# zhaoruiyang98/eftpipe

Hardware: AMD Instinct MI355X
Metric: theory P_l(k) evaluations/sec (single tracer, Nk=512, l=0,2,4) (higher is better)
Workload: dtype f64

## Files before the change

### eftpipe_amd/csrc/eftb_kernels.hpp

```cpp
#pragma once
#include <hip/hip_runtime.h>
#include <stdint.h>
#include <stdlib.h>

namespace eftb {

constexpr int NS = 80;
constexpr int NPOW = 257;
constexpr int NHALF = 128;
constexpr int NCH = 129;

constexpr int NROW = 24;

typedef double v4d __attribute__((ext_vector_type(4)));
typedef double v2d __attribute__((ext_vector_type(2)));

__device__ __forceinline__ void xcd_decode(int ntile, int& tile, int& group) {
    const int flat = blockIdx.x, ng = gridDim.x / ntile;
    if ((ng & 7) == 0) {
        const int slot = flat >> 3;
        tile = slot % ntile;
        group = (flat & 7) + 8 * (slot / ntile);
    } else {
        tile = flat % ntile;
// ... 74 lines not shown
__device__ __forceinline__ void qf_body(int w, int nq, const double* __restrict__ fgrow, const double* __restrict__ Qpoly, double* __restrict__ Q) {
    const int tid = threadIdx.x;
    const double f = fgrow[w];
    for (int idx = tid; idx < 2 * nq; idx += blockDim.x) {
        const int a = idx / nq, rest = idx % nq;
        const double* c = Qpoly + ((size_t)(1 - a) * nq + rest) * 15;
        double cv[15];
#pragma unroll
        for (int p = 0; p < 15; ++p) cv[p] = c[p];
        const double f2 = f * f;
        double ev = cv[14], od = cv[13];
#pragma unroll
        for (int p = 12; p >= 0; p -= 2) {
            ev = fma(ev, f2, cv[p]);
            if (p >= 1) od = fma(od, f2, cv[p - 1]);
        }
        Q[(size_t)w * 2 * nq + idx] = fma(od, f, ev);
    }
}

__global__ __launch_bounds__(256) void prep_rows_qf_kernel(int B, PREP_ROWS_PARAMS, int nq, const double* __restrict__ fgrow,
                                                           const double* __restrict__ Qpoly, double* __restrict__ Q) {
    if ((int)blockIdx.x >= B) {
        qf_body(blockIdx.x - B, nq, fgrow, Qpoly, Q);
        return;
    }
    prep_rows_body<false>(PREP_ROWS_ARGS, 0, 0);
}

__global__ __launch_bounds__(256) void prep_rows_qf_lo_kernel(int B, PREP_ROWS_PARAMS, int nq, const double* __restrict__ fgrow,
                                                              const double* __restrict__ Qpoly, double* __restrict__ Q, int ntail_lo, int nxtail_lo) {
    if ((int)blockIdx.x >= B) {
        qf_body(blockIdx.x - B, nq, fgrow, Qpoly, Q);
        return;
    }
    prep_rows_body<true>(PREP_ROWS_ARGS, ntail_lo, nxtail_lo);
}
#undef PREP_ROWS_PARAMS
#undef PREP_ROWS_ARGS

constexpr int AD_T = NHALF + 2;
constexpr int AD_CH = 1;
constexpr int KSYN = 528;
constexpr int KLIN = 288;
constexpr int SYN_KPAD = 48;
constexpr int SYN_KC = 24;
static_assert(SYN_KPAD % SYN_KC == 0 && (32 * SYN_KC) % 256 == 0, "chunk must divide the padding and fill the staging threads");
constexpr int BAS22 = 8, BASC = 32;

__device__ __forceinline__ double readlane_f64(double v, int lane) {
    return __hiloint2double(__builtin_amdgcn_readlane(__double2hiint(v), lane), __builtin_amdgcn_readlane(__double2loint(v), lane));
}

template <int NC, int NW>
__global__ __launch_bounds__(64 * NW) void antidiag_kernel(int B, int Bmax, const double* __restrict__ coefT,
                                                           const double2* __restrict__ AD, double2* __restrict__ S) {
    constexpr int PB = 3, WPP = 2 * NC;
    static_assert(PB * WPP <= 64, "one wave-load must hold a block's weights");
    __shared__ double red[NW - 1][2 * NC][64];
    const int grp = blockIdx.y, jp = (grp & 1) ? NPOW - 1 - (int)blockIdx.x : (int)blockIdx.x;
    const int lane = threadIdx.x & 63, wave = threadIdx.x >> 6, w = grp * 64 + lane;
    const int wl = w < B ? w : B - 1;
    const int cnt = ((2 * NHALF + jp) >> 1) - jp + 1;
    const int per = (cnt + NW - 1) / NW, t0 = wave * per, t1 = min(cnt, t0 + per);
    const double* cr = coefT + wl;
    const double* ci = coefT + (size_t)NCH * Bmax + wl;
    double ar[NC], ai[NC];
#pragma unroll
    for (int q = 0; q < NC; ++q) ar[q] = ai[q] = 0.0;
    if (t0 < t1) {
        const double* adw = reinterpret_cast<const double*>(AD + ((size_t)jp * AD_T + t0) * NC);
        const int nw = (t1 - t0) * WPP;
        auto wload = [&](int blk) { return adw[min(blk * PB * WPP + lane, nw - 1)]; };
        double xr[PB], xi[PB], yr[PB], yi[PB];
        auto coef = [&](int t, int p) {
            const int n = jp + t, qn = n <= NHALF ? n : 2 * NHALF - n;
            xr[p] = cr[(size_t)qn * Bmax];
            xi[p] = ci[(size_t)qn * Bmax];
            yr[p] = cr[(size_t)t * Bmax];
            yi[p] = ci[(size_t)t * Bmax];
        };
        double wc = wload(0);
#pragma unroll
        for (int p = 0; p < PB; ++p) coef(min(t0 + p, t1 - 1), p);
        const int nblk = (t1 - t0 + PB - 1) / PB;
        for (int blk = 0; blk < nblk; ++blk) {
            const double wn = wload(blk + 1);
#pragma unroll
            for (int p = 0; p < PB; ++p) {
                const int t = t0 + blk * PB + p;
                const double on = t < t1 ? 1.0 : 0.0;
                const double xim = jp + t <= NHALF ? xi[p] : -xi[p], yim = -yi[p];
                const double pr = (xr[p] * yr[p] - xim * yim) * on, pi = (xr[p] * yim + xim * yr[p]) * on;
                __builtin_amdgcn_sched_barrier(0);
                coef(min(t + PB, t1 - 1), p);
                __builtin_amdgcn_sched_barrier(0);
#pragma unroll
                for (int q = 0; q < NC; ++q) {
                    const double mx = readlane_f64(wc, p * WPP + 2 * q), my = readlane_f64(wc, p * WPP + 2 * q + 1);
                    ar[q] = fma(mx, pr, fma(-my, pi, ar[q]));
                    ai[q] = fma(mx, pi, fma(my, pr, ai[q]));
                }
                __builtin_amdgcn_sched_barrier(0);
            }
            wc = wn;
        }
    }
    if (wave > 0) {
#pragma unroll
        for (int q = 0; q < NC; ++q) {
            red[wave - 1][2 * q][lane] = ar[q];
            red[wave - 1][2 * q + 1][lane] = ai[q];
        }
    }
    __syncthreads();
    if (wave == 0 && w < B) {
#pragma unroll
        for (int q = 0; q < NC; ++q) {
#pragma unroll
            for (int v = 0; v < NW - 1; ++v) {
                ar[q] += red[v][2 * q][lane];
                ai[q] += red[v][2 * q + 1][lane];
            }
            S[((size_t)w * NC + q) * NPOW + jp] = make_double2(ar[q], ai[q]);
        }
    }
}

template <int NC, int NW>
__global__ __launch_bounds__(64 * NW) void antidiag_nh_kernel(int B, int Bmax, const double* __restrict__ coefT,
                                                              const double2* __restrict__ AD, double2* __restrict__ S, int nh) {
    constexpr int PB = 3, WPP = 2 * NC;
    static_assert(PB * WPP <= 64, "one wave-load must hold a block's weights");
    __shared__ double red[NW - 1][2 * NC][64];
    const int npow = 2 * nh + 1, nch = nh + 1, adt = nh + 2;
    const int grp = blockIdx.y, jp = (grp & 1) ? npow - 1 - (int)blockIdx.x : (int)blockIdx.x;
    const int lane = threadIdx.x & 63, wave = threadIdx.x >> 6, w = grp * 64 + lane;
    const int wl = w < B ? w : B - 1;
    const int cnt = ((2 * nh + jp) >> 1) - jp + 1;
    const int per = (cnt + NW - 1) / NW, t0 = wave * per, t1 = min(cnt, t0 + per);
    const double* cr = coefT + wl;
    const double* ci = coefT + (size_t)nch * Bmax + wl;
    double ar[NC], ai[NC];
#pragma unroll
    for (int q = 0; q < NC; ++q) ar[q] = ai[q] = 0.0;
    if (t0 < t1) {
        const double* adw = reinterpret_cast<const double*>(AD + ((size_t)jp * adt + t0) * NC);
        const int nw = (t1 - t0) * WPP;
        auto wload = [&](int blk) { return adw[min(blk * PB * WPP + lane, nw - 1)]; };
        double xr[PB], xi[PB], yr[PB], yi[PB];
        auto coef = [&](int t, int p) {
            const int n = jp + t, qn = n <= nh ? n : 2 * nh - n;
            xr[p] = cr[(size_t)qn * Bmax];
            xi[p] = ci[(size_t)qn * Bmax];
            yr[p] = cr[(size_t)t * Bmax];
            yi[p] = ci[(size_t)t * Bmax];
        };
        double wc = wload(0);
#pragma unroll
        for (int p = 0; p < PB; ++p) coef(min(t0 + p, t1 - 1), p);
        const int nblk = (t1 - t0 + PB - 1) / PB;
        for (int blk = 0; blk < nblk; ++blk) {
            const double wn = wload(blk + 1);
#pragma unroll
            for (int p = 0; p < PB; ++p) {
                const int t = t0 + blk * PB + p;
                const double on = t < t1 ? 1.0 : 0.0;
                const double xim = jp + t <= nh ? xi[p] : -xi[p], yim = -yi[p];
                const double pr = (xr[p] * yr[p] - xim * yim) * on, pi = (xr[p] * yim + xim * yr[p]) * on;
                __builtin_amdgcn_sched_barrier(0);
                coef(min(t + PB, t1 - 1), p);
                __builtin_amdgcn_sched_barrier(0);
#pragma unroll
                for (int q = 0; q < NC; ++q) {
                    const double mx = readlane_f64(wc, p * WPP + 2 * q), my = readlane_f64(wc, p * WPP + 2 * q + 1);
                    ar[q] = fma(mx, pr, fma(-my, pi, ar[q]));
                    ai[q] = fma(mx, pi, fma(my, pr, ai[q]));
                }
                __builtin_amdgcn_sched_barrier(0);
            }
            wc = wn;
        }
    }
    if (wave > 0) {
#pragma unroll
        for (int q = 0; q < NC; ++q) {
            red[wave - 1][2 * q][lane] = ar[q];
            red[wave - 1][2 * q + 1][lane] = ai[q];
        }
    }
    __syncthreads();
    if (wave == 0 && w < B) {
#pragma unroll
        for (int q = 0; q < NC; ++q) {
#pragma unroll
            for (int v = 0; v < NW - 1; ++v) {
                ar[q] += red[v][2 * q][lane];
                ai[q] += red[v][2 * q + 1][lane];
            }
            S[((size_t)w * NC + q) * npow + jp] = make_double2(ar[q], ai[q]);
        }
    }
}

template <int NC>
__global__ __launch_bounds__(64) void build_rows_kernel(int sets, int Bmax, int Nl, int nlc, int nb, const double* __restrict__ coef,
                                                         const double2* __restrict__ S, const double2* __restrict__ mlj,
                                                         const double2* __restrict__ linvec, double* __restrict__ A22,
                                                         double* __restrict__ A13, double* __restrict__ ACF, double* __restrict__ ALC) {
    const int w = blockIdx.x, cf = blockIdx.y, jp = blockIdx.z * 64 + threadIdx.x;
    if (((sets >> cf) & 1) && jp < NPOW) {
        double zr[NC], zi[NC];
#pragma unroll
        for (int q = 0; q < NC; ++q) {
            zr[q] = zi[q] = 0.0;
#pragma unroll
            for (int ch = 0; ch < AD_CH; ++ch) {
                const double2 v = S[(((size_t)ch * Bmax + w) * NC + q) * NPOW + jp];
                zr[q] += v.x;
                zi[q] += v.y;
            }
        }
        const int o0 = jp == 0 ? 0 : 2 * jp - 1;
        if (cf == 0) {
#pragma unroll
            for (int q = 0; q < NC; ++q)
                if (q < nb) {
                    double* o = A22 + ((size_t)w * BAS22 + q) * KSYN;
                    o[o0] = zr[q];
                    if (jp) o[o0 + 1] = zi[q];
                }
        } else {
            for (int l = 0; l < Nl; ++l) {
                const double2 m = mlj[l * NPOW + jp];
#pragma unroll
                for (int q = 0; q < NC; ++q) {
                    double* o = ACF + ((size_t)w * BASC + l * NC + q) * KSYN;
                    o[o0] = m.x * zr[q] - m.y * zi[q];
                    if (jp) o[o0 + 1] = m.x * zi[q] + m.y * zr[q];
                }
            }
        }
    }
    if ((sets >> (2 + cf)) & 1) {
        const int nrows = cf == 0 ? 10 : nlc * Nl, v0 = cf == 0 ? 0 : 10;
        double* out = cf == 0 ? A13 + (size_t)w * 10 * KLIN : ALC + (size_t)w * nlc * Nl * KLIN;
        const double* c = coef + (size_t)w * 2 * NCH;
        for (int e = jp; e < nrows * NCH; e += 320) {
            const int row = e / NCH, mp = e % NCH, n = NHALF - mp;
            const double2 v = linvec[(size_t)(v0 + row) * NCH + n];
            const double cr = c[n], ci = n == NHALF ? 0.0 : c[NCH + n];
            double* o = out + (size_t)row * KLIN;
            if (mp == 0) o[0] = cr * v.x - ci * v.y;
            else {
                o[2 * mp - 1] = cr * v.x - ci * v.y;
// ... 4175 lines not shown
```

### eftpipe_amd/csrc/eftbird.hip

```cpp
#include "../../include/eftbird.h"

#include <hip/hip_runtime.h>
#include <dlfcn.h>
#include <rccl/rccl.h>

#include <algorithm>
#include <array>
#include <atomic>
#include <chrono>
#include <cmath>
#include <condition_variable>
#include <mutex>
#include <thread>
#include <cstdarg>
#include <cstdint>
#include <cstdio>
#include <cstdlib>
#include <cstring>
#include <functional>
#include <memory>
#include <string>
#include <tuple>
#include <algorithm>
#include <vector>
// ... 333 lines not shown
    ncclResult_t (*Send)(const void*, size_t, ncclDataType_t, int, ncclComm_t, hipStream_t) = nullptr;
    ncclResult_t (*Recv)(void*, size_t, ncclDataType_t, int, ncclComm_t, hipStream_t) = nullptr;
    const char* (*GetErrorString)(ncclResult_t) = nullptr;
};
static RcclApi g_rccl;

static int rccl_load() {
    if (g_rccl.handle) return 0;
    void* h = dlopen("librccl.so.1", RTLD_NOW | RTLD_GLOBAL);
    if (!h) h = dlopen("librccl.so", RTLD_NOW | RTLD_GLOBAL);
    if (!h) return fail("cannot load librccl.so: %s", dlerror());
#define RSYM(field, name)                                                 \
    g_rccl.field = reinterpret_cast<decltype(g_rccl.field)>(dlsym(h, name)); \
    if (!g_rccl.field) return fail("librccl.so lacks %s", name);
    RSYM(GetUniqueId, "ncclGetUniqueId")
    RSYM(CommInitRank, "ncclCommInitRank")
    RSYM(CommDestroy, "ncclCommDestroy")
    RSYM(GroupStart, "ncclGroupStart")
    RSYM(GroupEnd, "ncclGroupEnd")
    RSYM(Send, "ncclSend")
    RSYM(Recv, "ncclRecv")
    RSYM(GetErrorString, "ncclGetErrorString")
#undef RSYM
    g_rccl.handle = h;
    return 0;
}

#define NCCLCHK(expr)                                                                            \
    do {                                                                                         \
        ncclResult_t _r = (expr);                                                                \
        if (_r != ncclSuccess) return fail("%s failed: %s", #expr, g_rccl.GetErrorString(_r));   \
    } while (0)

static inline void trace_point(eftb_engine* e, int p, hipStream_t st) {
    if (e->trace_slot >= 0) (void)hipEventRecord(e->evTrace[e->trace_slot][p], st);
}

static inline size_t kpad(int n) { return (size_t)(n + SYN_KPAD - 1) / SYN_KPAD * SYN_KPAD; }

static inline int cfg_nh(const eftb_config& c) { return c.nfft ? c.nfft / 2 : NHALF; }
static inline int cfg_npow(const eftb_config& c) { return 2 * cfg_nh(c) + 1; }
static inline int cfg_nch(const eftb_config& c) { return cfg_nh(c) + 1; }

static size_t need_table_bytes(const eftb_config& c, int id) {
    const size_t D = sizeof(double);
    const int Nn = 2 * c.NIR * c.Na;
    switch (id) {
        case EFTB_T_K: return D * c.Nk;
        case EFTB_T_S: return D * NS;
        case EFTB_T_LNKIN: return D * c.Nkin;
        case EFTB_T_SKT: return D * kpad(c.Nkin) * c.Nk;
        case EFTB_T_GCT: case EFTB_T_ECT: return D * kpad(c.Nkin + c.ntail) * 2 * cfg_nch(c);
        case EFTB_T_LNXTAIL: return D * c.ntail;
        case EFTB_T_AD: return 2 * D * (size_t)(c.nbasis + (c.with_resum ? c.nbasis13 : 0)) * cfg_npow(c) * (cfg_nh(c) + 2);
        case EFTB_T_EXP22: return D * 28 * BAS22;
        case EFTB_T_EXPC: return c.with_resum ? D * (size_t)c.Nl * 38 * BASC : 0;
        case EFTB_T_MLJ: return c.with_resum ? 2 * D * c.Nl * cfg_npow(c) : 0;
        case EFTB_T_LINVEC: return 2 * D * (size_t)(10 + (c.with_resum ? (c.with_nnlo ? 3 : 2) * c.Nl : 0)) * cfg_nch(c);
        case EFTB_T_SYNK: return D * (size_t)ksyn_of(cfg_nh(c)) * c.Nk;
        case EFTB_T_LINK: return D * (size_t)klin_of(cfg_nh(c)) * c.Nk;
        case EFTB_T_SYNS: return c.with_resum ? D * (size_t)ksyn_of(cfg_nh(c)) * NS : 0;
        case EFTB_T_LINS: return c.with_resum ? D * (size_t)klin_of(cfg_nh(c)) * NS : 0;
        case EFTB_T_L11: return D * c.Nl * 3;
        case EFTB_T_LCT: return D * c.Nl * 6;
        case EFTB_T_L22: return D * c.Nl * 28;
        case EFTB_T_L13: return D * c.Nl * 10;
        case EFTB_T_GRP: return sizeof(int32_t) * 38 * 2;
        case EFTB_T_BXT: return c.with_resum ? D * kpad(c.Nkin + c.nxtail) * 2 * NS : 0;
        case EFTB_T_TYT: return 0;
        case EFTB_T_LNXXTAIL: return c.with_resum ? D * c.nxtail : 0;
        case EFTB_T_WQLAST2: return c.with_resum ? D * (c.nxtail_lo ? 4 : 2) : 0;
        case EFTB_T_QPOLY: return c.with_resum ? D * 2 * c.Nl * c.Nl * Nn * 15 : 0;
        case EFTB_T_H: return c.with_resum ? D * c.Na * NS * c.Nk : 0;
        case EFTB_T_RSBASIS: case EFTB_T_RSBASISS: return c.with_resum ? D * RS_NB * 16 : 0;
        case EFTB_T_RSROWS: return c.with_resum ? sizeof(int32_t) * 2 * RS3_ROWS : 0;
        case EFTB_T_MU: case EFTB_T_WMU: return c.with_ap ? D * c.nmu : 0;
        case EFTB_T_LEGMU: return c.with_ap ? D * c.Nl * c.nmu : 0;
        case EFTB_T_SPBAND: return c.with_ap ? D * (size_t)(2 * SPL_HB + 1) * c.Nk : 0;
        case EFTB_T_SPCBAND: return c.with_ap ? D * (size_t)(2 * SPL_HB + 1) * c.Nk : 0;
        case EFTB_T_SPLOCAL: return c.with_ap ? D * (size_t)16 * c.Nk : 0;
        case EFTB_T_APFID: return c.with_ap ? D * 2 : 0;
        case EFTB_T_LCTN: return c.with_nnlo ? D * c.Nl * 6 : 0;
        case EFTB_T_BAO: return c.optiresum && c.with_resum ? D * (2 * NS + 4) : 0;
        case EFTB_T_GCT2: case EFTB_T_GCT2T: return c.dual_coef ? D * kpad(c.Nkin + c.ntail) * 2 * cfg_nch(c) : 0;
        case EFTB_T_QEPOLY: return c.with_resum && c.Nl == 3 ? D * 2 * c.Nl * c.Nl * RSD_NN * 15 : 0;
    }
    return 0;
}

static size_t need_buffer_elems(const eftb_config& c, int id) {
    const size_t B = c.max_batch;
    const int Nn = 2 * c.NIR * c.Na;
    switch (id) {
        case EFTB_B_PIN: return B * c.Nkin;
        case EFTB_B_F: case EFTB_B_DA: case EFTB_B_H: return B;
        case EFTB_B_P11: return B * c.Nk;
        case EFTB_B_P22: return B * 28 * c.Nk;
        case EFTB_B_P13: return B * 10 * c.Nk;
        case EFTB_B_C11: case EFTB_B_CCT: return c.with_resum ? B * c.Nl * NS : 0;
        case EFTB_B_CC: return c.with_resum ? B * c.Nl * 38 * NS : 0;
        case EFTB_B_CLOOPL: return c.with_resum ? B * c.Nl * 12 * NS : 0;
        case EFTB_B_TEMPL: return B * c.Nl * NROW * c.Nk;
        case EFTB_B_XY: return c.with_resum ? B * 2 * NS : 0;
        case EFTB_B_Q: return c.with_resum ? B * 2 * c.Nl * c.Nl * Nn : 0;
        case EFTB_B_BIAS: return B * NROW;
        case EFTB_B_PLK: return B * c.Nl * c.Nk;
        case EFTB_B_COEF: return B * 2 * cfg_nch(c);
// ... 2 lines not shown
        case EFTB_B_CCTN: return c.with_nnlo && c.with_resum ? B * c.Nl * NS : 0;
        case EFTB_B_TEMPLN: return c.with_nnlo ? B * c.Nl * NROW * c.Nk : 0;
        case EFTB_B_BIASN: return c.with_nnlo ? B * 3 : 0;
        case EFTB_B_GROWSN: return c.with_nnlo ? B * MARG_NG1 * 3 : 0;
    }
    return 0;
}

template <typename T>
static inline const T* tb(const eftb_engine* e, int id) { return static_cast<const T*>(e->tab[id]); }

static void queue_synth(SynthBatch& sb, const double* A, long long a_group, int groups, int rpg, int K, const double* Tab, int X, double* out,
                        long long o_group, const double* gscale, const double* xscale) {
    SynthDesc& d = sb.p[sb.n];
    d.A = A; d.Tab = Tab; d.out = out; d.gscale = gscale; d.xscale = xscale;
    d.a_group = a_group; d.o_group = o_group; d.M = groups * rpg; d.rpg = rpg; d.K = K; d.X = X;
    d.wgx = (X + 63) / 64;
    d.wg_end = (sb.n ? sb.p[sb.n - 1].wg_end : 0) + d.wgx * ((d.M + 31) / 32);
    ++sb.n;
}

static void launch_synth(hipStream_t st, const SynthBatch& sb) {
    if (sb.n) hipLaunchKernelGGL(synth_kernel, dim3(sb.p[sb.n - 1].wg_end), dim3(256), 0, st, sb);
}

static void launch_gemm_direct(hipStream_t st, SynthBatch sb) {
    int end = 0;
    for (int i = 0; i < sb.n; ++i) {
        SynthDesc& d = sb.p[i];
        d.wgx = (d.X + 31) / 32;
        end += d.wgx * ((d.M + 15) / 16);
        d.wg_end = end;
    }
    if (sb.n) hipLaunchKernelGGL((gemm_direct_kernel<4>), dim3(end), dim3(256), 0, st, sb);
}

template <typename... P, typename... A>
static void launch_nh(void (*fixed)(P...), void (*any)(P..., int), int nh, dim3 grid, dim3 block, hipStream_t st, A... args) {
    if (nh == NHALF) hipLaunchKernelGGL(fixed, grid, block, 0, st, args...);
    else hipLaunchKernelGGL(any, grid, block, 0, st, args..., nh);
}

template <typename... P, typename... A>
static void launch_two(void (*one)(P...), void (*two)(P...), int J1, dim3 grid, dim3 block, size_t lds, hipStream_t st, A... args) {
    if (J1 > 64) hipLaunchKernelGGL(two, grid, block, lds, st, args...);
    else hipLaunchKernelGGL(one, grid, block, lds, st, args...);
}

static void launch_antidiag_rows(eftb_engine* e, hipStream_t st, int B, int sets, const double* coef, const double* coefT, bool contracted = false) {
    const eftb_config& c = e->c;
    const int nc = c.nbasis + (c.with_resum ? c.nbasis13 : 0);
    const int nh = cfg_nh(c), npow = 2 * nh + 1;
    const dim3 grid(npow, (B + 63) / 64), rgrid(B, 2, (npow + 63) / 64);
#define AD_ARGS B, c.max_batch, coefT, tb<double2>(e, EFTB_T_AD), e->SAD
#define ROW_ARGS sets, c.max_batch, c.Nl, c.with_nnlo ? 3 : 2, c.nbasis, coef, e->SAD, tb<double2>(e, EFTB_T_MLJ), tb<double2>(e, EFTB_T_LINVEC), e->A22, e->A13, \
                 e->ACF, e->ALC
#define PLK_ARGS c.max_batch, c.nbasis, coef, e->SAD, tb<double2>(e, EFTB_T_MLJ), tb<double2>(e, EFTB_T_LINVEC), e->buf[EFTB_B_BIAS], e->buf[EFTB_B_F], \
                 tb<double>(e, EFTB_T_L11), tb<double>(e, EFTB_T_LCT), tb<double>(e, EFTB_T_L22), tb<double>(e, EFTB_T_L13), tb<int>(e, EFTB_T_GRP), \
                 tb<double>(e, EFTB_T_EXP22), tb<double>(e, EFTB_T_EXPC), e->A22, e->A13, e->ACF, e->ALC
    if ((sets & 0x10) && !(contracted && WHATIF_SKIP(4))) {
        if (nc == 9) launch_nh(antidiag_kernel<9, 2>, antidiag_nh_kernel<9, 2>, nh, grid, dim3(128), st, AD_ARGS);
        else launch_nh(antidiag_kernel<7, 2>, antidiag_nh_kernel<7, 2>, nh, grid, dim3(128), st, AD_ARGS);
    }
    if (contracted) trace_point(e, 11, st);
    if (contracted && nc == 9) {
        if (!WHATIF_SKIP(8)) launch_nh(build_rows_plk_kernel<9>, build_rows_plk_nh_kernel<9>, nh, rgrid, dim3(64), st, PLK_ARGS);
    } else if (nc == 9) launch_nh(build_rows_kernel<9>, build_rows_nh_kernel<9>, nh, rgrid, dim3(64), st, ROW_ARGS);
    else launch_nh(build_rows_kernel<7>, build_rows_nh_kernel<7>, nh, rgrid, dim3(64), st, ROW_ARGS);
#undef AD_ARGS
#undef ROW_ARGS
#undef PLK_ARGS
}

static int launch_operator(eftb_engine* e, int id, int B, int t0 = 0, int tstride = 1, bool commit = true) {
    if (id < 0 || id >= (int)e->ops.size()) return fail("operator id %d out of range", id);
    const eftb_engine::Op& o = e->ops[id];
    if (o.nl_in != e->cur_nl || o.nx_in != e->cur_nx)
        return fail("operator %d expects templates [%d][24][%d], the block is [%d][24][%d]", id, o.nl_in, o.nx_in, e->cur_nl, e->cur_nx);
    auto launch = [&](const eftb_engine::Op& m, int r0, int nr) {
        GemmDesc g{};
        const long long bin = (long long)o.nl_in * NROW * o.nx_in, bout = (long long)o.nl_out * NROW * o.nx_out;
        g.A = e->buf[EFTB_B_TEMPL] + (size_t)t0 * bin + (size_t)r0 * o.nx_in; g.a_group = bin * tstride; g.a_row = o.nx_in;
        g.a_seg = (long long)NROW * o.nx_in;
        g.rows = ((B - t0 + tstride - 1) / tstride) * nr; g.rows_per_group = nr; g.nseg = o.nl_in; g.kseg = o.nx_in;
        g.B = m.dev; g.ldb = m.ld; g.ncols = o.nl_out * o.nx_out;
        g.C = e->Talt + (size_t)t0 * bout + (size_t)r0 * o.nx_out; g.c_group = bout * tstride; g.c_row = o.nx_out;
        g.c_colgroup = (long long)NROW * o.nx_out;
        g.cols_per_group = o.nx_out;
        if (g.ncols <= 16 * GN_MAXT)
            hipLaunchKernelGGL(gemm_narrow_kernel, dim3((g.rows + 15) / 16, 1), dim3(256), 0, (e->opstream ? e->opstream : e->stream), g, GemmZ{});
        else
            hipLaunchKernelGGL(gemm_rows_kernel, dim3((g.rows + 63) / 64, (g.ncols + 255) / 256), dim3(256), GEMM_LDS, (e->opstream ? e->opstream : e->stream), g);
    };
    if (o.st_op < 0) launch(o, 0, NROW);
    else {
        launch(o, 0, NROW - 3);
        launch(e->ops[o.st_op], NROW - 3, 3);
    }
    if (!commit) return 0;
    std::swap(e->buf[EFTB_B_TEMPL], e->Talt);
    e->cur_nl = o.nl_out;
    e->cur_nx = o.nx_out;
    return 0;
}

static int launch_pipeline_operator(eftb_engine* e, int B) {
    if (e->tracer_ops.empty()) {
// ... 3629 lines not shown
```

### eftpipe_amd/engine.py

```python
from __future__ import annotations

import ctypes as C
import os

import numpy as np

from . import _lib as L
from .tables import EngineConfig, build_tables

NROW = 24
ROWS = dict(P11l=slice(0, 3), Pctl=slice(3, 9), Ploopl=slice(9, 21), Pstl=slice(21, 24))


class Engine:
    def __init__(self, cfg: EngineConfig, max_batch: int = 1, device: int = 0, loop_cache=None, coalesce: int = 1):
        self.lib = L.load()
        self.cfg = cfg
        t = self.tables = build_tables(cfg, loop_cache)
        self.Nl, self.Nk, self.Nkin = cfg.Nl, t["k"].size, t["kin"].size
        self.k, self.kin, self.s = t["k"], t["kin"], t["s"]
        self.max_batch = int(max_batch)
        self.dims = (cfg.Nl, self.Nk)
        self._op_shapes = []
        self._pipeline_op = -1
        self.ntracers = 1
        self._tracer_ops = []
        self._latency_mode = os.environ.get("EFTB_LATENCY_MODE", "1") != "0"
        self._plk_direct = False
        self._step_ptr, self._step_n, self._views = C.c_void_p(), C.c_size_t(), {}
        c = L.Config()
        c.device, c.Nl, c.Nk, c.Nkin, c.max_batch = device, cfg.Nl, self.Nk, self.Nkin, self.max_batch * max(1, int(coalesce))
        c.step_batch = self.max_batch if coalesce > 1 else 0
        c.with_resum, c.with_ap, c.ap_stochastic = int(cfg.with_resum), int(cfg.with_ap), int(cfg.APst)
        c.nmu = cfg.nbinsmu
        c.ntail = t["lnx_tail"].size
        c.nbasis = t["comb22"].shape[1]
        c.nbasis13 = t["comb13"].shape[1] if cfg.with_resum else 0
        if cfg.with_resum:
            c.nxtail = t["lnx_xtail"].size
            c.NIR, c.Na, c.Nklow = (int(x) for x in t["resum_dims"])
        c.with_nnlo = int(cfg.with_NNLO)
        c.dual_coef = int("Gc2" in t)
        c.optiresum = int(cfg.optiresum and cfg.with_resum)
        c.nfft = 0 if cfg.NFFT == 256 else int(cfg.NFFT)
        c.ntail_lo = int(t["ntail_lo"])
        c.nxtail_lo = int(t.get("nxtail_lo", 0))
        self._cconf = c
        h = C.c_void_p()
        L.check(self.lib.eftb_create(C.byref(c), C.byref(h)))
        self._h = h
        self._upload(t)
        L.check(self.lib.eftb_finalize(self._h))

    def _set(self, name, arr, dtype=np.float64):
        a = np.ascontiguousarray(arr, dtype=dtype)
        L.check(self.lib.eftb_set_table(self._h, L.T[name], a.ctypes.data_as(C.c_void_p), a.nbytes))

    def _upload(self, t):
        cfg = self.cfg
        self._set("K", t["k"])
        self._set("S", t["s"])
        self._set("LNKIN", np.log(t["kin"]))
        kpad = lambda n: (n + 47) // 48 * 48
        Nkin, ntail = t["kin"].size, t["lnx_tail"].size
        nch = t["Gc"].shape[1]

        def stack_gc(G, E):
            out = np.zeros((kpad(Nkin + ntail), 2 * nch))
            for c_ in range(2):
                out[:Nkin, c_ * nch : (c_ + 1) * nch] = G[c_].T
                out[Nkin : Nkin + ntail, c_ * nch : (c_ + 1) * nch] = E[c_].T
            return out

        skt = np.zeros((kpad(Nkin), self.Nk))
        skt[:Nkin] = t["Sk"].T
        self._set("SKT", skt)
        gct = stack_gc(t["Gc"], t["Ec"])
        self._set("GCT", gct)
        self._set("ECT", gct.T)
        self._set("LNXTAIL", t["lnx_tail"])
        cplx = lambda z: np.stack([z.real, z.imag], axis=-1)
        self._set("AD", cplx(t["ad"].transpose(1, 2, 0)))
        exp22 = np.zeros((28, 8))
        exp22[:, : t["comb22"].shape[1]] = t["comb22"]
        self._set("EXP22", exp22)
        self._set("LINVEC", cplx(t["linvec"]))
        self._set("SYNK", t["syn_k"])
        self._set("LINK", t["lin_k"])
        for n in ("L11", "LCT", "L22", "L13"):
            self._set(n, t[n.lower()])
        self._set("GRP", np.concatenate([t["grp22"], t["grp13"]]), np.int32)
        if cfg.with_NNLO:
            self._set("LCTN", t["lctn"])
        if "bao" in t:
            self._set("BAO", t["bao"])
        if "Gc2" in t:
            gct2 = stack_gc(t["Gc2"], t["Ec2"])
            self._set("GCT2", gct2)
            self._set("GCT2T", gct2.T)
        if cfg.with_resum:
            expc = np.zeros((cfg.Nl * 38, 32))
            expc[:, : t["expand_c"].shape[1]] = t["expand_c"]
            self._set("EXPC", expc)
            self._set("MLJ", cplx(t["mlj"]))
            self._set("SYNS", t["syn_s"])
            self._set("LINS", t["lin_s"])
            nxt = t["lnx_xtail"].size
            bxt = np.zeros((kpad(Nkin + nxt), 2 * 80))
            bxt[:Nkin, :80], bxt[:Nkin, 80:] = t["BX"].T, t["BY"].T
            bxt[Nkin : Nkin + nxt, :80], bxt[Nkin : Nkin + nxt, 80:] = t["TX"].T, t["TY"].T
            self._set("BXT", bxt)
            self._set("LNXXTAIL", t["lnx_xtail"])
            self._set("WQLAST2", t["wq_last2"])
            self._set("QPOLY", t["Qpoly"])
            if "QEpoly" in t:
                self._set("QEPOLY", t["QEpoly"])
            self._set("H", t["H"].transpose(0, 2, 1))
            if "rs_rows" in t:
                self._set("RSBASIS", t["rs_basis"])
                self._set("RSBASISS", t["rs_basis_scaled"])
                self._set("RSROWS", t["rs_rows"], np.int32)
        if cfg.with_ap:
            self._set("MU", t["mu"])
            self._set("WMU", t["wmu"])
            self._set("LEGMU", t["legmu"])
            self._set("SPBAND", t["sp_band"])
            self._set("SPCBAND", t["sp_cband"])
            self._set("SPLOCAL", t["sp_local"])
            self._set("APFID", t["ap_fid"])

    def set_ap_fiducial(self, DA, H):
        self._set("APFID", np.array([DA, H], dtype=np.float64))

    def set_graph_replay(self, flag):
        L.check(self.lib.eftb_set_option(self._h, 2, int(bool(flag))))

    def set_check_finite(self, flag):
        L.check(self.lib.eftb_set_option(self._h, 3, int(bool(flag))))

    def time_dominant(self, every):
        L.check(self.lib.eftb_set_option(self._h, 4, int(every)))

    def time_kernels(self, which):
        L.check(self.lib.eftb_set_option(self._h, 7, int(which)))

    def kernel_time(self, kind, reset=True, cosmologies=False):
        ms, n, nc = C.c_double(), C.c_longlong(), C.c_longlong()
        L.check(self.lib.eftb_kernel_time_ex(self._h, int(kind), C.byref(ms), C.byref(n), C.byref(nc), int(bool(reset))))
        return (ms.value, n.value, nc.value) if cosmologies else (ms.value, n.value)

    def dominant_time(self, reset=True):
        ms, n = C.c_double(), C.c_longlong()
# ... 381 lines not shown
```

### eftpipe_amd/tables.py

```python
from __future__ import annotations

from dataclasses import dataclass, field
from typing import Optional

import numpy as np
from scipy.interpolate import CubicSpline
from scipy.special import legendre, spherical_jn

from . import loopmath as lm

NS = 80
NPOW = 257
NHALF = 128
NFFT_MIN, NFFT_MAX = 256, 512


def check_nfft(NFFT):
    if NFFT % 2 or NFFT < NFFT_MIN or NFFT > NFFT_MAX:
        raise ValueError(f"NFFT={NFFT} unsupported: the HIP engine takes even values from {NFFT_MIN} to {NFFT_MAX}")


def edge_window(N, window):
    if window is None:
        w = np.ones(N + 1)
# ... 29 lines not shown
        tilt = np.exp(-bias * i * self.dx)
        phase = np.exp(-2j * np.pi * (((m[:, None] - N // 2) * i[None, :]) % N) / N)
        D = phase * (coef_factor * edge_window(N, window))[:, None]
        if xin is not None:
            S = CubicSpline(xin, np.eye(len(xin)), axis=0, extrapolate=False)(self.x[lo:hi])
            t = tilt[lo:hi]
            if kernel is not None:
                t = t * kernel(self.x[lo:hi])
            self.G = D[:, lo:hi] @ (t[:, None] * S)
        self.low_active = extrap[0] == "extrap" and xin[0] > self.x[0]
        self.high_active = extrap[1] == "extrap" and xin[-1] < self.x[-1]
        self.E_lo = D[:, :lo] * tilt[:lo] if self.low_active else np.zeros((N + 1, 0), complex)
        self.E_hi = D[:, hi:] * tilt[hi:] if self.high_active else np.zeros((N + 1, 0), complex)
        self.lnx_lo = np.log(self.x[:lo]) if self.low_active else np.zeros(0)
        self.lnx_hi = np.log(self.x[hi:]) if self.high_active else np.zeros(0)


def loop_basis(M22, tol=1e-11):
    from scipy.linalg import qr

    A = M22.reshape(M22.shape[0], -1)
    _, Rq, piv = qr(A.T, mode="economic", pivoting=True)
    d = np.abs(np.diag(Rq))
    rank = int(np.sum(d > tol * d[0]))
    basis = np.sort(piv[:rank])
    X = np.linalg.lstsq(A[basis].T, A.T, rcond=None)[0].T
    resid = np.max(np.abs(X @ A[basis] - A)) / np.max(np.abs(A))
    if resid > 1e-13 or np.max(np.abs(X.imag)) > 1e-12 or rank > 16:
        raise ValueError(f"loop-matrix basis reduction failed: rank {rank}, residual {resid:.2e}")
    X = X.real
    A = A[:, ::4]
    R = A.astype(np.clongdouble) - X.astype(np.longdouble) @ A[basis].astype(np.clongdouble)
    Ar = np.concatenate([A[basis].real, A[basis].imag], axis=1)
    X = X + np.linalg.lstsq(Ar.T, np.concatenate([R.real, R.imag], axis=1).astype(np.float64).T, rcond=None)[0].T
    return basis, np.ascontiguousarray(X)


def antidiagonal_tables(M22b, M13b):
    npow = np.shape(M22b)[-1]
    N = npow - 1
    mats = [np.asarray(M22b)]
    if M13b is not None:
        mats.append(np.asarray(M13b)[:, :, None] * np.ones((1, 1, npow)))
    M = np.concatenate(mats)
    Ms = M + np.swapaxes(M, 1, 2)
    idx = np.arange(npow)
    Ms[:, idx, idx] = M[:, idx, idx]
    AD = np.zeros((M.shape[0], npow, N // 2 + 2), dtype=complex)
    for jp in range(npow):
        cnt = ((N + jp) >> 1) - jp + 1
        tt = np.arange(cnt)
        AD[:, jp, :cnt] = Ms[:, jp + tt, N - tt]
    return AD


def synthesis_table(lnx, power, dpow, nharm, sign):
    K = 1 + 2 * nharm
    out = np.zeros(((K + 47) // 48 * 48, lnx.size))
    amp = np.exp(power * lnx)
    out[0] = amp
    j = np.arange(1, nharm + 1)
    th = dpow * np.outer(j, lnx)
    out[1:K:2] = 2.0 * amp * np.cos(th)
    out[2:K:2] = -sign * 2.0 * amp * np.sin(th)
    return out


def spline_factors(x):
    x = np.asarray(x, dtype=float)
    n = x.size
    dx = np.diff(x)
    lower, diag, upper = np.zeros(n), np.zeros(n), np.zeros(n)
    diag[1:-1] = 2.0 * (dx[:-1] + dx[1:])
    upper[1:-1] = dx[:-1]
    lower[1:-1] = dx[1:]
    diag[0], upper[0] = dx[1], x[2] - x[0]
    diag[-1], lower[-1] = dx[-2], x[-1] - x[-3]
    inv, cp = np.zeros(n), np.zeros(n)
    piv = diag[0]
    inv[0], cp[0] = 1.0 / piv, upper[0] / piv
    for i in range(1, n):
        piv = diag[i] - lower[i] * cp[i - 1]
        inv[i] = 1.0 / piv
        cp[i] = upper[i] / piv
    return dict(dx=dx, lower=lower, inv=inv, cp=cp)


SPL_HB = 32


def spline_derivative_band(x):
    x = np.asarray(x, dtype=float)
    n = x.size
    S = CubicSpline(x, np.eye(n), axis=0)(x, 1)
    band = np.zeros((2 * SPL_HB + 1, n))
    for d in range(2 * SPL_HB + 1):
        j = np.arange(n) + d - SPL_HB
        ok = (j >= 0) & (j < n)
        band[d, ok] = S[np.arange(n)[ok], j[ok]]
    return band


def bspline_tables(x):
    from scipy.interpolate import BSpline, make_interp_spline

    x = np.asarray(x, dtype=float)
# ... 121 lines not shown
        raise ValueError(f"unexpected IRcutoff option: {ircut}")
    if ircut and cfg.kIR is None:
        raise ValueError("kIR must be specified when doing IRcutoff")
    icut = int(np.searchsorted(kin, cfg.kIR)) if ircut else 0

    def cut_operator(N, xmin, xmax, bias, window):
        o = FFTLogOperator(N, xmin, xmax, bias, kin[icut:], window, extrap=("padding", "extrap"))
        o.G = np.hstack([np.zeros((o.G.shape[0], icut), dtype=complex), o.G])
        return o

    op = FFTLogOperator(NFFT, 1.5e-5, 1000.0, -1.6, kin, cfg.fft_window)
    nch = nh + 1
    op_cut = cut_operator(NFFT, 1.5e-5, 1000.0, -1.6, cfg.fft_window) if ircut else None
    op_k = op_cut if ircut in ("all", "loop") else op
    op_s = op_cut if ircut in ("all", "resum") else op
    ntail_lo = op.lnx_lo.size if (op_k is op or op_s is op) else 0

    def tail_op(o):
        E = np.hstack([op.E_hi[:nch], o.E_lo[:nch] if o.low_active else np.zeros((nch, ntail_lo), complex)])
        return np.ascontiguousarray(np.stack([E.real, E.imag]))

    t["Gc"] = np.ascontiguousarray(np.stack([op_k.G[:nch].real, op_k.G[:nch].imag]))
    t["Ec"] = tail_op(op_k)
    if op_s is not op_k:
        t["Gc2"] = np.ascontiguousarray(np.stack([op_s.G[:nch].real, op_s.G[:nch].imag]))
        t["Ec2"] = tail_op(op_s)
    t["lnx_tail"] = np.concatenate([op.lnx_hi, op.lnx_lo[:ntail_lo]])
    t["ntail_lo"] = ntail_lo
    Pow = op.Pow
    nu = -0.5 * Pow
    if loop_cache is not None:
        if np.shape(loop_cache["Pow"]) != Pow.shape or np.any(np.asarray(loop_cache["Pow"]) != Pow):
            raise ValueError("loop-matrix cache was written for a different FFTLog configuration")
        M22, M13 = np.asarray(loop_cache["M22"]), np.asarray(loop_cache["M13"])
        if M22.shape != (28, npow, npow) or M13.shape != (10, npow):
            raise ValueError("loop-matrix cache has the wrong shapes")
    else:
        M22 = lm.matrices_22(nu)
        M13 = lm.vectors_13(nu)
    ells = 2 * np.arange(Nl)
    basis, comb = loop_basis(M22)
    t["basis22"], t["comb22"] = basis.astype(np.int32), comb
    vecs = [M13]
    if cfg.with_resum:
        basis13, comb13 = loop_basis(M13)
        t["comb13"] = comb13
        nb, nb13 = comb.shape[1], comb13.shape[1]
        expc = np.zeros((Nl * 38, Nl * (nb + nb13)))
        for l in range(Nl):
            expc[l * 28 : (l + 1) * 28, l * (nb + nb13) : l * (nb + nb13) + nb] = comb
            expc[Nl * 28 + l * 10 : Nl * 28 + (l + 1) * 10, l * (nb + nb13) + nb : (l + 1) * (nb + nb13)] = comb13
        t["expand_c"] = expc
        t["ad"] = antidiagonal_tables(M22[basis], M13[basis13])
        jp = np.arange(npow)
        t["mlj"] = lm.bessel_weight(ells[:, None], -op.bias - 0.5j * op.dpow * jp[None, :] - 1.5)
        if loop_cache is not None and np.shape(loop_cache["Mcf11"]) == (Nl, npow):
            vecs += [np.asarray(loop_cache["Mcf11"]), np.asarray(loop_cache["Mcfct"])]
        else:
            vecs += [lm.bessel_weight(ells[:, None], nu[None, :]), lm.bessel_weight(ells[:, None], nu[None, :] - 1.0)]
        if cfg.with_NNLO:
            if loop_cache is not None and np.shape(loop_cache.get("McfctNNLO")) == (Nl, npow):
                vecs.append(np.asarray(loop_cache["McfctNNLO"]))
            else:
                vecs.append(lm.bessel_weight(ells[:, None], nu[None, :] - 2.0))
        t["syn_s"] = synthesis_table(np.log(s), -2.0 * op.bias - 6.0, op.dpow, NFFT, sign=-1.0)
        t["lin_s"] = synthesis_table(np.log(s), -op.bias - 3.0, op.dpow, nh, sign=+1.0)
    else:
        t["ad"] = antidiagonal_tables(M22[basis], None)
    t["linvec"] = np.ascontiguousarray(np.concatenate(vecs)[:, :nch])
    if cfg.with_NNLO:
        t["lctn"] = np.concatenate([w["lctNNLO"], np.zeros((Nl, 3))], axis=1)
    t["syn_k"] = synthesis_table(np.log(k), 3.0 + 2.0 * op.bias, op.dpow, NFFT, sign=+1.0)
    t["lin_k"] = synthesis_table(np.log(k), 3.0 + op.bias, op.dpow, nh, sign=-1.0)

    if cfg.with_resum:
        NIR = 16 if Nl == 3 else 8
        Na = 3 if Nl == 3 else 2
        kr_mask = k >= 0.02
        kr = k[kr_mask]
        rop = FFTLogOperator(cfg.NFFT_resum, 0.1, 10000.0, -0.6, s[sr_idx], cfg.resum_window, extrap=("padding", "padding"))
        rM = np.stack([8.0 * np.pi**3 * lm.bessel_weight(2 * l, -0.5 * rop.Pow) for l in range(Na)])
        rk = np.exp(np.outer(-rop.Pow - 3.0, np.log(kr)))
        H = np.zeros((Na, Nk, NS))
        for v in range(Na):
            H[np.ix_([v], np.where(kr_mask)[0], sr_idx)] = np.real((rM[v][:, None] * rk).T @ rop.G)[None]
        t["H"] = H
        if cfg.optiresum:
            t["bao"] = bao
        wq = np.exp(-(kin**2) / cfg.LambdaIR**2) / kin**2
        xop = (cut_operator(32, 1.5e-5, 10.0, -2.6, cfg.irf_window) if ircut in ("all", "resum")
               else FFTLogOperator(32, 1.5e-5, 10.0, -2.6, kin, cfg.irf_window))
        XM = np.stack([lm.bessel_weight(2 * l, -0.5 * xop.Pow) for l in range(2)])
        XsPow = np.exp(np.outer(-xop.Pow - 3.0, np.log(s)))
        K = lambda D: np.real(np.einsum("ln,ns,ni->lsi", XM, XsPow, D))
        soff = cfg.irf_soffset ** (-xop.Pow - 3.0)
        Koff = lambda D: np.real(np.einsum("n,ni->i", XM[0] * soff, D))
        Ex = np.hstack([xop.E_hi, xop.E_lo])
        body, tail = K(xop.G), K(Ex)
        boff, toff = Koff(xop.G), Koff(Ex)
        t["BX"] = np.ascontiguousarray(cfg.irf_rescale * 2.0 / 3.0 * (boff[None, :] - body[0] - body[1]) * wq[None, :])
        t["BY"] = np.ascontiguousarray(2.0 * body[1] * wq[None, :])
        t["TX"] = np.ascontiguousarray(cfg.irf_rescale * 2.0 / 3.0 * (toff[None, :] - tail[0] - tail[1]))
        t["TY"] = np.ascontiguousarray(2.0 * tail[1])
        t["lnx_xtail"] = np.concatenate([xop.lnx_hi, xop.lnx_lo])
        t["nxtail_lo"] = xop.lnx_lo.size
        t["wq_last2"] = np.concatenate([wq[-2:], wq[:2]]) if xop.low_active else wq[-2:].copy()
        t["Qpoly"] = lm.q_polynomials(Nl)
        t["resum_dims"] = np.array([NIR, Na, int(np.sum(~kr_mask))], dtype=np.int32)
        t.update(resum_mfma_tables(t["Qpoly"], NIR, Na))
        if Nl == 3:
            t.update(resum_plk_tables(t["Qpoly"], NIR, Na))

    if cfg.with_ap:
        mu = np.linspace(0.0, 1.0, cfg.nbinsmu)
        wmu = np.full(cfg.nbinsmu, mu[1] - mu[0])
        wmu[0] = wmu[-1] = 0.5 * (mu[1] - mu[0])
        t["mu"], t["wmu"] = mu, wmu
        t["legmu"] = np.ascontiguousarray(((2 * ells + 1) / 2.0)[:, None] * legendre_table(Nl, mu))
        t["sp_band"] = spline_derivative_band(k)
        t["sp_cband"], t["sp_local"], _ = bspline_tables(k)
        t["ap_fid"] = np.array([cfg.DA_AP, cfg.H_AP], dtype=np.float64)
# ... 310 lines not shown
```

Before: 1.899 million.

## Compress antidiagonal 22-loop weights into a rank-4 real span with per-jp mixing

The 22-loop basis matrices along each antidiagonal are factored into at most four real weight columns, chosen by pivoted QR, plus a small complex mixing matrix per jp. Gamma-ratio factors are folded into the ECT coefficient tables so the weights become real. The kernel then does real FMAs over 4 accumulators instead of complex FMAs over 7 basis entries, uses PB=4, and applies the mixing in the epilogue. This cuts readlanes, FLOPs and weight bandwidth in the hot loop. In exchange it adds host-side high-precision table construction and a numerical low-rank assumption that must hold to f64 accuracy.

```diff
diff --git a/eftpipe_amd/csrc/eftb_kernels.hpp b/eftpipe_amd/csrc/eftb_kernels.hpp
--- a/eftpipe_amd/csrc/eftb_kernels.hpp
+++ b/eftpipe_amd/csrc/eftb_kernels.hpp
@@ -150,88 +150,20 @@
     return __hiloint2double(__builtin_amdgcn_readlane(__double2hiint(v), lane), __builtin_amdgcn_readlane(__double2loint(v), lane));
 }
 
+constexpr int AD_NB = 7;
+constexpr int AD_NQ = 4;
+constexpr int AD_HDR = 2 * AD_NB * AD_NQ;
+__host__ __device__ constexpr int ad_wpp(int nc) { return AD_NQ + 2 * (nc - AD_NB); }
+__host__ __device__ constexpr size_t ad_record(int nc, int nh) { return AD_HDR + (size_t)(nh + 2) * ad_wpp(nc); }
+
 template <int NC, int NW>
-__global__ __launch_bounds__(64 * NW) void antidiag_kernel(int B, int Bmax, const double* __restrict__ coefT,
-                                                           const double2* __restrict__ AD, double2* __restrict__ S) {
-    constexpr int PB = 3, WPP = 2 * NC;
-    static_assert(PB * WPP <= 64, "one wave-load must hold a block's weights");
-    __shared__ double red[NW - 1][2 * NC][64];
-    const int grp = blockIdx.y, jp = (grp & 1) ? NPOW - 1 - (int)blockIdx.x : (int)blockIdx.x;
-    const int lane = threadIdx.x & 63, wave = threadIdx.x >> 6, w = grp * 64 + lane;
-    const int wl = w < B ? w : B - 1;
-    const int cnt = ((2 * NHALF + jp) >> 1) - jp + 1;
-    const int per = (cnt + NW - 1) / NW, t0 = wave * per, t1 = min(cnt, t0 + per);
-    const double* cr = coefT + wl;
-    const double* ci = coefT + (size_t)NCH * Bmax + wl;
-    double ar[NC], ai[NC];
-#pragma unroll
-    for (int q = 0; q < NC; ++q) ar[q] = ai[q] = 0.0;
-    if (t0 < t1) {
-        const double* adw = reinterpret_cast<const double*>(AD + ((size_t)jp * AD_T + t0) * NC);
-        const int nw = (t1 - t0) * WPP;
-        auto wload = [&](int blk) { return adw[min(blk * PB * WPP + lane, nw - 1)]; };
-        double xr[PB], xi[PB], yr[PB], yi[PB];
-        auto coef = [&](int t, int p) {
-            const int n = jp + t, qn = n <= NHALF ? n : 2 * NHALF - n;
-            xr[p] = cr[(size_t)qn * Bmax];
-            xi[p] = ci[(size_t)qn * Bmax];
-            yr[p] = cr[(size_t)t * Bmax];
-            yi[p] = ci[(size_t)t * Bmax];
-        };
-        double wc = wload(0);
-#pragma unroll
-        for (int p = 0; p < PB; ++p) coef(min(t0 + p, t1 - 1), p);
-        const int nblk = (t1 - t0 + PB - 1) / PB;
-        for (int blk = 0; blk < nblk; ++blk) {
-            const double wn = wload(blk + 1);
-#pragma unroll
-            for (int p = 0; p < PB; ++p) {
-                const int t = t0 + blk * PB + p;
-                const double on = t < t1 ? 1.0 : 0.0;
-                const double xim = jp + t <= NHALF ? xi[p] : -xi[p], yim = -yi[p];
-                const double pr = (xr[p] * yr[p] - xim * yim) * on, pi = (xr[p] * yim + xim * yr[p]) * on;
-                __builtin_amdgcn_sched_barrier(0);
-                coef(min(t + PB, t1 - 1), p);
-                __builtin_amdgcn_sched_barrier(0);
-#pragma unroll
-                for (int q = 0; q < NC; ++q) {
-                    const double mx = readlane_f64(wc, p * WPP + 2 * q), my = readlane_f64(wc, p * WPP + 2 * q + 1);
-                    ar[q] = fma(mx, pr, fma(-my, pi, ar[q]));
-                    ai[q] = fma(mx, pi, fma(my, pr, ai[q]));
-                }
-                __builtin_amdgcn_sched_barrier(0);
-            }
-            wc = wn;
-        }
-    }
-    if (wave > 0) {
-#pragma unroll
-        for (int q = 0; q < NC; ++q) {
-            red[wave - 1][2 * q][lane] = ar[q];
-            red[wave - 1][2 * q + 1][lane] = ai[q];
-        }
-    }
-    __syncthreads();
-    if (wave == 0 && w < B) {
-#pragma unroll
-        for (int q = 0; q < NC; ++q) {
-#pragma unroll
-            for (int v = 0; v < NW - 1; ++v) {
-                ar[q] += red[v][2 * q][lane];
-                ai[q] += red[v][2 * q + 1][lane];
-            }
-            S[((size_t)w * NC + q) * NPOW + jp] = make_double2(ar[q], ai[q]);
-        }
-    }
-}
-
-template <int NC, int NW>
-__global__ __launch_bounds__(64 * NW) void antidiag_nh_kernel(int B, int Bmax, const double* __restrict__ coefT,
-                                                              const double2* __restrict__ AD, double2* __restrict__ S, int nh) {
-    constexpr int PB = 3, WPP = 2 * NC;
-    static_assert(PB * WPP <= 64, "one wave-load must hold a block's weights");
-    __shared__ double red[NW - 1][2 * NC][64];
-    const int npow = 2 * nh + 1, nch = nh + 1, adt = nh + 2;
+__device__ __forceinline__ void antidiag_body(int B, int Bmax, const double* __restrict__ coefT, const double* __restrict__ AD,
+                                              double2* __restrict__ S, const int nh) {
+    constexpr int NM = NC - AD_NB, NA = AD_NQ + NM;
+    constexpr int PB = 4, WPP = ad_wpp(NC);
+    static_assert(NM >= 0 && PB * WPP <= 64, "one wave-load must hold a block's weights");
+    __shared__ double red[NW - 1][2 * NA][64];
+    const int npow = 2 * nh + 1, nch = nh + 1;
     const int grp = blockIdx.y, jp = (grp & 1) ? npow - 1 - (int)blockIdx.x : (int)blockIdx.x;
     const int lane = threadIdx.x & 63, wave = threadIdx.x >> 6, w = grp * 64 + lane;
     const int wl = w < B ? w : B - 1;
@@ -239,11 +171,12 @@
     const int per = (cnt + NW - 1) / NW, t0 = wave * per, t1 = min(cnt, t0 + per);
     const double* cr = coefT + wl;
     const double* ci = coefT + (size_t)nch * Bmax + wl;
-    double ar[NC], ai[NC];
-#pragma unroll
-    for (int q = 0; q < NC; ++q) ar[q] = ai[q] = 0.0;
+    const double* rec = AD + (size_t)jp * ad_record(NC, nh);
+    double ar[NA], ai[NA];
+#pragma unroll
+    for (int q = 0; q < NA; ++q) ar[q] = ai[q] = 0.0;
     if (t0 < t1) {
-        const double* adw = reinterpret_cast<const double*>(AD + ((size_t)jp * adt + t0) * NC);
+        const double* adw = rec + AD_HDR + (size_t)t0 * WPP;
         const int nw = (t1 - t0) * WPP;
         auto wload = [&](int blk) { return adw[min(blk * PB * WPP + lane, nw - 1)]; };
         double xr[PB], xi[PB], yr[PB], yi[PB];
@@ -270,10 +203,16 @@
                 coef(min(t + PB, t1 - 1), p);
                 __builtin_amdgcn_sched_barrier(0);
 #pragma unroll
-                for (int q = 0; q < NC; ++q) {
-                    const double mx = readlane_f64(wc, p * WPP + 2 * q), my = readlane_f64(wc, p * WPP + 2 * q + 1);
-                    ar[q] = fma(mx, pr, fma(-my, pi, ar[q]));
-                    ai[q] = fma(mx, pi, fma(my, pr, ai[q]));
+                for (int q = 0; q < AD_NQ; ++q) {
+                    const double f = readlane_f64(wc, p * WPP + q);
+                    ar[q] = fma(f, pr, ar[q]);
+                    ai[q] = fma(f, pi, ai[q]);
+                }
+#pragma unroll
+                for (int q = 0; q < NM; ++q) {
+                    const double mx = readlane_f64(wc, p * WPP + AD_NQ + 2 * q), my = readlane_f64(wc, p * WPP + AD_NQ + 2 * q + 1);
+                    ar[AD_NQ + q] = fma(mx, pr, fma(-my, pi, ar[AD_NQ + q]));
+                    ai[AD_NQ + q] = fma(mx, pi, fma(my, pr, ai[AD_NQ + q]));
                 }
                 __builtin_amdgcn_sched_barrier(0);
             }
@@ -282,7 +221,7 @@
     }
     if (wave > 0) {
 #pragma unroll
-        for (int q = 0; q < NC; ++q) {
+        for (int q = 0; q < NA; ++q) {
             red[wave - 1][2 * q][lane] = ar[q];
             red[wave - 1][2 * q + 1][lane] = ai[q];
         }
@@ -290,15 +229,40 @@
     __syncthreads();
     if (wave == 0 && w < B) {
 #pragma unroll
-        for (int q = 0; q < NC; ++q) {
+        for (int q = 0; q < NA; ++q) {
 #pragma unroll
             for (int v = 0; v < NW - 1; ++v) {
                 ar[q] += red[v][2 * q][lane];
                 ai[q] += red[v][2 * q + 1][lane];
             }
-            S[((size_t)w * NC + q) * npow + jp] = make_double2(ar[q], ai[q]);
-        }
-    }
+        }
+        const double2* C = reinterpret_cast<const double2*>(rec);
+#pragma unroll
+        for (int b = 0; b < AD_NB; ++b) {
+            double sr = 0.0, si = 0.0;
+#pragma unroll
+            for (int q = 0; q < AD_NQ; ++q) {
+                const double2 c = C[b * AD_NQ + q];
+                sr = fma(c.x, ar[q], fma(-c.y, ai[q], sr));
+                si = fma(c.x, ai[q], fma(c.y, ar[q], si));
+            }
+            S[((size_t)w * NC + b) * npow + jp] = make_double2(sr, si);
+        }
+#pragma unroll
+        for (int q = 0; q < NM; ++q) S[((size_t)w * NC + AD_NB + q) * npow + jp] = make_double2(ar[AD_NQ + q], ai[AD_NQ + q]);
+    }
+}
+
+template <int NC, int NW>
+__global__ __launch_bounds__(64 * NW) void antidiag_kernel(int B, int Bmax, const double* __restrict__ coefT,
+                                                           const double* __restrict__ AD, double2* __restrict__ S) {
+    antidiag_body<NC, NW>(B, Bmax, coefT, AD, S, NHALF);
+}
+
+template <int NC, int NW>
+__global__ __launch_bounds__(64 * NW) void antidiag_nh_kernel(int B, int Bmax, const double* __restrict__ coefT,
+                                                              const double* __restrict__ AD, double2* __restrict__ S, int nh) {
+    antidiag_body<NC, NW>(B, Bmax, coefT, AD, S, nh);
 }
 
 template <int NC>
diff --git a/eftpipe_amd/csrc/eftbird.hip b/eftpipe_amd/csrc/eftbird.hip
--- a/eftpipe_amd/csrc/eftbird.hip
+++ b/eftpipe_amd/csrc/eftbird.hip
@@ -409,7 +409,7 @@
         case EFTB_T_SKT: return D * kpad(c.Nkin) * c.Nk;
         case EFTB_T_GCT: case EFTB_T_ECT: return D * kpad(c.Nkin + c.ntail) * 2 * cfg_nch(c);
         case EFTB_T_LNXTAIL: return D * c.ntail;
-        case EFTB_T_AD: return 2 * D * (size_t)(c.nbasis + (c.with_resum ? c.nbasis13 : 0)) * cfg_npow(c) * (cfg_nh(c) + 2);
+        case EFTB_T_AD: return D * cfg_npow(c) * ad_record(c.nbasis + (c.with_resum ? c.nbasis13 : 0), cfg_nh(c));
         case EFTB_T_EXP22: return D * 28 * BAS22;
         case EFTB_T_EXPC: return c.with_resum ? D * (size_t)c.Nl * 38 * BASC : 0;
         case EFTB_T_MLJ: return c.with_resum ? 2 * D * c.Nl * cfg_npow(c) : 0;
@@ -518,7 +518,7 @@
     const int nc = c.nbasis + (c.with_resum ? c.nbasis13 : 0);
     const int nh = cfg_nh(c), npow = 2 * nh + 1;
     const dim3 grid(npow, (B + 63) / 64), rgrid(B, 2, (npow + 63) / 64);
-#define AD_ARGS B, c.max_batch, coefT, tb<double2>(e, EFTB_T_AD), e->SAD
+#define AD_ARGS B, c.max_batch, coefT, tb<double>(e, EFTB_T_AD), e->SAD
 #define ROW_ARGS sets, c.max_batch, c.Nl, c.with_nnlo ? 3 : 2, c.nbasis, coef, e->SAD, tb<double2>(e, EFTB_T_MLJ), tb<double2>(e, EFTB_T_LINVEC), e->A22, e->A13, \
                  e->ACF, e->ALC
 #define PLK_ARGS c.max_batch, c.nbasis, coef, e->SAD, tb<double2>(e, EFTB_T_MLJ), tb<double2>(e, EFTB_T_LINVEC), e->buf[EFTB_B_BIAS], e->buf[EFTB_B_F], \
diff --git a/eftpipe_amd/engine.py b/eftpipe_amd/engine.py
--- a/eftpipe_amd/engine.py
+++ b/eftpipe_amd/engine.py
@@ -75,12 +75,17 @@
         skt = np.zeros((kpad(Nkin), self.Nk))
         skt[:Nkin] = t["Sk"].T
         self._set("SKT", skt)
+        def times_gd(gT):
+            z = (gT[:nch] + 1j * gT[nch:]) * t["ad_gd"][:, None]
+            return np.concatenate([z.real, z.imag])
+
         gct = stack_gc(t["Gc"], t["Ec"])
         self._set("GCT", gct)
-        self._set("ECT", gct.T)
+        self._set("ECT", times_gd(gct.T))
         self._set("LNXTAIL", t["lnx_tail"])
         cplx = lambda z: np.stack([z.real, z.imag], axis=-1)
-        self._set("AD", cplx(t["ad"].transpose(1, 2, 0)))
+        npow = t["ad_w"].shape[0]
+        self._set("AD", np.concatenate([cplx(t["ad_c"]).reshape(npow, -1), t["ad_w"].reshape(npow, -1)], axis=1))
         exp22 = np.zeros((28, 8))
         exp22[:, : t["comb22"].shape[1]] = t["comb22"]
         self._set("EXP22", exp22)
@@ -97,7 +102,7 @@
         if "Gc2" in t:
             gct2 = stack_gc(t["Gc2"], t["Ec2"])
             self._set("GCT2", gct2)
-            self._set("GCT2T", gct2.T)
+            self._set("GCT2T", times_gd(gct2.T))
         if cfg.with_resum:
             expc = np.zeros((cfg.Nl * 38, 32))
             expc[:, : t["expand_c"].shape[1]] = t["expand_c"]
diff --git a/eftpipe_amd/tables.py b/eftpipe_amd/tables.py
--- a/eftpipe_amd/tables.py
+++ b/eftpipe_amd/tables.py
@@ -105,6 +105,60 @@
         tt = np.arange(cnt)
         AD[:, jp, :cnt] = Ms[:, jp + tt, N - tt]
     return AD
+
+
+AD_NQ = 4
+
+
+def antidiagonal_span_tables(nu, basis, M13b):
+    import mpmath
+    from scipy.linalg import qr
+
+    nu = np.asarray(nu)
+    npow = nu.size
+    N = npow - 1
+    nb = len(basis)
+    ld = np.longdouble
+    with mpmath.workdps(34):
+        mnu = [mpmath.mpc(float(v.real), float(v.imag)) for v in nu]
+        mgd = [mpmath.gamma(1.5 - v) / mpmath.gamma(v) / (v * (1 + v) * (2 * v - 1)) for v in mnu]
+        mh = [mpmath.gamma(v + mnu[N] - 1.5) / (8 * mpmath.pi**1.5 * mpmath.gamma(3 - v - mnu[N])) for v in mnu]
+        gd = np.array([complex(v) for v in mgd])
+        h_hi = np.array([complex(v) for v in mh])
+        h_lo = np.array([complex(v - mpmath.mpc(w.real, w.imag)) for v, w in zip(mh, h_hi)])
+    h = h_hi.astype(np.clongdouble) + h_lo.astype(np.clongdouble)
+    d = lm.formula_data()["M22b"]
+    Dn = nu * (1.0 + nu) * (2.0 * nu - 1.0)
+    DD = Dn[:, None] * Dn[None, :]
+    Nb = np.stack([lm._rational(d[int(b)], (nu[:, None], nu[None, :])) * DD for b in basis])
+    n13 = 0 if M13b is None else np.shape(M13b)[0]
+    W = np.zeros((npow, N // 2 + 2, AD_NQ + 2 * n13))
+    Cm = np.zeros((npow, nb, AD_NQ), dtype=np.clongdouble)
+    for jp in range(npow):
+        cnt = ((N + jp) >> 1) - jp + 1
+        tt = np.arange(cnt)
+        n, m = jp + tt, N - tt
+        pw = np.where(n < m, 2.0, 1.0)
+        Y = Nb[:, n, m] * pw[None, :]
+        Y = np.concatenate([Y.real, Y.imag])
+        sc = 1.0 / np.max(np.abs(Nb[:, n, m]), axis=0)
+        Ys = Y * sc[None, :]
+        _, Rq, piv = qr(Ys.T, mode="economic", pivoting=True)
+        dg = np.abs(np.diag(Rq))
+        r = min(AD_NQ, int(np.sum(dg > 1e-10 * dg[0])))
+        sel = np.sort(piv[:r])
+        W[jp, :cnt, :r] = Y[sel].T
+        A = Ys[sel].T
+        X = np.linalg.lstsq(A, Ys.T, rcond=None)[0]
+        R = Ys.T.astype(ld) - A.astype(ld) @ X.astype(ld)
+        X = X.astype(ld) + np.linalg.lstsq(A, R.astype(np.float64), rcond=None)[0].astype(ld)
+        Cm[jp, :, :r] = (X[:, :nb] + 1j * X[:, nb:]).T * h[jp]
+        if n13:
+            V = np.asarray(M13b)
+            w13 = np.where(n < m, V[:, n] + V[:, m], V[:, n]) / (gd[n] * gd[m])[None, :]
+            W[jp, :cnt, AD_NQ::2] = w13.real.T
+            W[jp, :cnt, AD_NQ + 1 :: 2] = w13.imag.T
+    return dict(ad_w=W, ad_c=Cm.astype(np.complex128), ad_gd=np.ascontiguousarray(gd[: N // 2 + 1]))
 
 
 def synthesis_table(lnx, power, dpow, nharm, sign):
@@ -332,6 +386,7 @@
             expc[Nl * 28 + l * 10 : Nl * 28 + (l + 1) * 10, l * (nb + nb13) + nb : (l + 1) * (nb + nb13)] = comb13
         t["expand_c"] = expc
         t["ad"] = antidiagonal_tables(M22[basis], M13[basis13])
+        t.update(antidiagonal_span_tables(nu, basis, M13[basis13]))
         jp = np.arange(npow)
         t["mlj"] = lm.bessel_weight(ells[:, None], -op.bias - 0.5j * op.dpow * jp[None, :] - 1.5)
         if loop_cache is not None and np.shape(loop_cache["Mcf11"]) == (Nl, npow):
@@ -347,6 +402,7 @@
         t["lin_s"] = synthesis_table(np.log(s), -op.bias - 3.0, op.dpow, nh, sign=+1.0)
     else:
         t["ad"] = antidiagonal_tables(M22[basis], None)
+        t.update(antidiagonal_span_tables(nu, basis, None))
     t["linvec"] = np.ascontiguousarray(np.concatenate(vecs)[:, :nch])
     if cfg.with_NNLO:
         t["lctn"] = np.concatenate([w["lctNNLO"], np.zeros((Nl, 3))], axis=1)
```

Result: slower. 1.867 million (-1.7%).
